# zdebruine/MMVAE

Hardware: AMD Instinct MI355X
Metric: cells/sec per MMVAE train step (higher is better)
Workload: dtype f32; 1 GPU; c2: 2-modality MMVAE train step, 20000 genes each, latent 128, K=1, batch 512/GPU, adversarial=False; global_batch=512, parallelism=dp1, exchange=none

## Files before the change

__graft_entry__.py:

```python
import os
import subprocess
import sys

ROOT = os.path.dirname(os.path.abspath(__file__))
if ROOT not in sys.path:
    sys.path.insert(0, ROOT)


def build() -> None:
    csrc = os.path.join(ROOT, "mmvae_amd", "csrc")
    subprocess.run(["make", "-C", csrc, "-j4"], check=True)
    from mmvae_amd import _lib

    lib = _lib.load()
    assert lib.mmvae_abi_version() >= 1 and lib.mmvae_build_arch() == b"gfx950"
    from mmvae_amd import _stats_lib

    stats = _stats_lib.load_stats()
    assert stats.mmvae_stats_abi_version() == _stats_lib.STATS_ABI_VERSION and stats.mmvae_stats_build_arch() == b"gfx950"
    from mmvae_amd import _disc_lib

    disc = _disc_lib.load_disc()
    assert disc.mmvae_disc_abi_version() == _disc_lib.DISC_ABI_VERSION and disc.mmvae_disc_build_arch() == b"gfx950"
    from mmvae_amd import _umap_lib

    um = _umap_lib.load_umap()
    assert um.mmvae_umap_abi_version() == _umap_lib.UMAP_ABI_VERSION and um.mmvae_umap_build_arch() == b"gfx950"
    from mmvae_amd import _hist_lib

    hist = _hist_lib.load_hist()
    assert hist.mmvae_hist_abi_version() == _hist_lib.HIST_ABI_VERSION and hist.mmvae_hist_build_arch() == b"gfx950"
    from mmvae_amd import _prep_lib

    prep = _prep_lib.load_prep()
    assert prep.mmvae_prep_abi_version() == _prep_lib.PREP_ABI_VERSION and prep.mmvae_prep_build_arch() == b"gfx950"
    from mmvae_amd import data

    assert data.feed_lib().mmvae_feed_abi_version() == 3
    import mmvae_amd.models
    import mmvae_amd.modules
    import mmvae_amd.engine


def smoke() -> None:
    import torch

    assert torch.cuda.is_available(), "smoke() needs a GPU"
    from mmvae_amd import _lib

    _lib.load()
# ... 12 lines not shown
```

mmvae_amd/csrc/elbo_optim.hip:

```cpp
#include "common.h"

namespace {

__global__ __launch_bounds__(256) void reparam_kl_fwd_kernel(int B, int Z, int K, const float* __restrict__ mu,
                                                             const float* __restrict__ a_raw,
                                                             const float* __restrict__ eps, float var_eps,
                                                             float* __restrict__ std_out, float* __restrict__ z_out,
                                                             float* __restrict__ kl_row, float* __restrict__ stat_row) {
    const int lane = threadIdx.x & 63;
    const int b = blockIdx.x * 4 + (threadIdx.x >> 6);
    if (b >= B) return;
    float kl = 0.f, smu = 0.f, svar = 0.f;
    for (int j = lane; j < Z; j += 64) {
        const int64_t o = (int64_t)b * Z + j;
        const float m = mu[o];
        const float v = expf(a_raw[o]) + var_eps;
        const float s = sqrtf(v);
        if (std_out) std_out[o] = s;
        const float vr = s * s;
        kl += 0.5f * (vr + m * m - 1.f - logf(vr));
        smu += m;
        svar += vr;
        if (z_out)
            for (int k = 0; k < K; ++k) {
// ... 366 lines not shown
        for (int64_t i = threadIdx.x; i < n; i += 1024) s += (double)row[i];
        __syncthreads();
        red[threadIdx.x] = s;
        __syncthreads();
        for (int st = 512; st >= 1; st >>= 1) {
            if ((int)threadIdx.x < st) red[threadIdx.x] += red[threadIdx.x + st];
            __syncthreads();
        }
        const float r = (float)red[0];
        if (threadIdx.x == 0 && out_each) out_each[h] = r;
        total = h == 0 ? r : total + r;
    }
    if (threadIdx.x == 0 && out_total) out_total[0] = total;
}

constexpr int64_t SQN_CHUNK = 1 << 16;

__device__ __forceinline__ float sqnorm_chunk(int64_t n, const float* __restrict__ g, int64_t chunk, float* red) {
    const int64_t beg = chunk * SQN_CHUNK;
    int64_t end = beg + SQN_CHUNK;
    if (end > n) end = n;
    float s = 0.f;
    const bool vec = ((reinterpret_cast<uintptr_t>(g) & 15u) == 0);
    if (vec) {
        const int64_t nv = (end - beg) / 4;
        const f32x4* gv = reinterpret_cast<const f32x4*>(g + beg);
        float s0 = 0.f, s1 = 0.f, s2 = 0.f, s3 = 0.f;
        int64_t i = threadIdx.x;
        for (; i + 7 * 256 < nv; i += 8 * 256) {
            f32x4 v[8];
#pragma unroll
            for (int u = 0; u < 8; ++u) v[u] = gv[i + u * 256];
#pragma unroll
            for (int u = 0; u < 8; ++u) {
                s0 += v[u].x * v[u].x;
                s1 += v[u].y * v[u].y;
                s2 += v[u].z * v[u].z;
                s3 += v[u].w * v[u].w;
            }
        }
        for (; i < nv; i += 256) {
            const f32x4 v = gv[i];
            s0 += v.x * v.x;
            s1 += v.y * v.y;
            s2 += v.z * v.z;
            s3 += v.w * v.w;
        }
        s = (s0 + s1) + (s2 + s3);
        for (int64_t i = beg + nv * 4 + threadIdx.x; i < end; i += 256) s += g[i] * g[i];
    } else {
        for (int64_t i = beg + threadIdx.x; i < end; i += 256) s += g[i] * g[i];
    }
    s = wave_sum(s);
    __syncthreads();
    if ((threadIdx.x & 63) == 0) red[threadIdx.x >> 6] = s;
    __syncthreads();
    return (red[0] + red[1]) + (red[2] + red[3]);
}

__global__ __launch_bounds__(256) void sqnorm_kernel(int64_t n, const float* __restrict__ g,
                                                     float* __restrict__ partials) {
    __shared__ float red[4];
    const float s = sqnorm_chunk(n, g, blockIdx.x, red);
    if (threadIdx.x == 0) partials[blockIdx.x] = s;
}

__device__ __forceinline__ void adam_prepare_body(int64_t np, const float* partials, float max_norm, float grad_scale,
                                                  float beta1, float beta2, float* __restrict__ state, unsigned flags,
                                                  double* red) {
    double s = 0.0;
    if (flags & MMVAE_PREPARE_NORM)
        for (int64_t i = threadIdx.x; i < np; i += 256) s += (double)partials[i];
    red[threadIdx.x] = s;
    __syncthreads();
    if (threadIdx.x == 0) {
        double t = 0.0;
        if (flags & MMVAE_PREPARE_NORM)
            for (int i = 0; i < 256; ++i) t += red[i];
        adam_state_finish(state, t, flags, max_norm, grad_scale, beta1, beta2);
    }
}

__global__ __launch_bounds__(256) void adam_prepare_kernel(int64_t np, const float* __restrict__ partials,
                                                           float max_norm, float grad_scale, float beta1, float beta2,
                                                           float* __restrict__ state, unsigned flags) {
    __shared__ double red[256];
    adam_prepare_body(np, partials, max_norm, grad_scale, beta1, beta2, state, flags, red);
}

struct SqRanges {
    const float* g[4];
    int64_t n[4];
    int nb[4];
    int nr;
};
// ... 12 lines not shown
    }
    const float s = sqnorm_chunk(r.n[k], r.g[k], b, red);
    if (threadIdx.x == 0) {
        partials[blockIdx.x] = s;
        __threadfence();
        last = atomicAdd(ticket, 1u) == gridDim.x - 1;
    }
    __syncthreads();
    if (!last) return;
    if (threadIdx.x == 0) *ticket = 0u;
    __threadfence();
    adam_prepare_body(np_all, const_cast<const float*>(reinterpret_cast<const volatile float*>(partials_all)), max_norm,
                      grad_scale, beta1, beta2, state, flags, dred);
}

#ifndef MMVAE_ADAM_NT
#define MMVAE_ADAM_NT 1
#endif
__device__ __forceinline__ void adam_one(float& p, float g, float& m, float& v, float gmul, float wd, float b1, float b2,
                                         float step_size, float inv_bc2_sqrt, float eps, float cv = 0.f) {
    const float gs = g * gmul;
    const float gc = (gs != gs ? gs : fminf(fmaxf(gs, -cv), cv)) + wd * p;
    g = g * gmul + wd * p;
    if (cv > 0.f) g = gc;
    m = m + (1.f - b1) * (g - m);
    v = b2 * v + (1.f - b2) * g * g;
    const float denom = sqrtf(v) * inv_bc2_sqrt + eps;
    p = p - step_size * (m / denom);
}

__device__ __forceinline__ float mul_uncontracted(float a, float b) {
#pragma clang fp contract(off)
    return a * b;
}
__device__ __forceinline__ void adam_hyper(const float* __restrict__ hyper, float& lr, float& wd, float& decay) {
    decay = 1.f;
    lr = hyper[0];
    wd = hyper[1];
    if (hyper[2] != 0.f) {
        decay = 1.f - mul_uncontracted(lr, wd);
        wd = 0.f;
    }
}
__device__ __forceinline__ void adam_elem(float& p, float g, float& m, float& v, float gmul, float wd, float decay,
                                          float b1, float b2, float step_size, float inv_bc2_sqrt, float eps, float cv) {
    p = mul_uncontracted(p, decay);
    adam_one(p, g, m, v, gmul, wd, b1, b2, step_size, inv_bc2_sqrt, eps, cv);
}

__device__ __forceinline__ void adam_step_body(int64_t n, float* __restrict__ p, const float* __restrict__ g,
                                               float* __restrict__ m, float* __restrict__ v,
                                               const float* __restrict__ state, const float* __restrict__ hyper,
                                               float b1, float b2, float eps, float grad_scale, int vec, int copy_n,
                                               const float* copy_src, float* copy_dst) {
    if (copy_n > 0 && blockIdx.x == 0)
        for (int i = threadIdx.x; i < copy_n; i += blockDim.x) copy_dst[i] = copy_src[i];
    float lr, wd, decay;
    adam_hyper(hyper, lr, wd, decay);
    const float gmul = state[2] * grad_scale;
    const float step_size = lr / state[3];
    const float inv_bc2_sqrt = 1.f / sqrtf(state[4]);
    const float cv = state[5];
    const int64_t stride = (int64_t)gridDim.x * blockDim.x;
    const int64_t tid0 = (int64_t)blockIdx.x * blockDim.x + threadIdx.x;
    if (vec) {
        const int64_t nv = n / 4;
        f32x4* pv = reinterpret_cast<f32x4*>(p);
        const f32x4* gv = reinterpret_cast<const f32x4*>(g);
        f32x4* mv = reinterpret_cast<f32x4*>(m);
        f32x4* vv = reinterpret_cast<f32x4*>(v);
        for (int64_t i = tid0; i < nv; i += stride) {
#if MMVAE_ADAM_NT
            f32x4 pp = MMVAE_ADAM_NT == 2 ? __builtin_nontemporal_load(pv + i) : pv[i];
            f32x4 gg = __builtin_nontemporal_load(gv + i), mm = __builtin_nontemporal_load(mv + i),
                  vw = __builtin_nontemporal_load(vv + i);
#else
            f32x4 pp = pv[i], gg = gv[i], mm = mv[i], vw = vv[i];
#endif
#pragma unroll
            for (int e = 0; e < 4; ++e) {
                float pe = pp[e], me = mm[e], ve = vw[e];
                adam_elem(pe, gg[e], me, ve, gmul, wd, decay, b1, b2, step_size, inv_bc2_sqrt, eps, cv);
                pp[e] = pe;
                mm[e] = me;
                vw[e] = ve;
            }
#if MMVAE_ADAM_NT == 2
            __builtin_nontemporal_store(pp, pv + i);
#else
            pv[i] = pp;
#endif
#if MMVAE_ADAM_NT
            __builtin_nontemporal_store(mm, mv + i);
            __builtin_nontemporal_store(vw, vv + i);
#else
            mv[i] = mm;
            vv[i] = vw;
#endif
        }
        for (int64_t i = nv * 4 + tid0; i < n; i += stride)
            adam_elem(p[i], g[i], m[i], v[i], gmul, wd, decay, b1, b2, step_size, inv_bc2_sqrt, eps, cv);
    } else {
        for (int64_t i = tid0; i < n; i += stride)
            adam_elem(p[i], g[i], m[i], v[i], gmul, wd, decay, b1, b2, step_size, inv_bc2_sqrt, eps, cv);
    }
}

__global__ __launch_bounds__(256) void adam_step_hp_kernel(int64_t n, float* __restrict__ p, const float* __restrict__ g,
                                                           float* __restrict__ m, float* __restrict__ v,
                                                           const float* __restrict__ state,
                                                           const float* __restrict__ hyper, float b1, float b2, float eps,
                                                           float grad_scale, int vec, int copy_n, const float* copy_src,
                                                           float* copy_dst) {
    adam_step_body(n, p, g, m, v, state, hyper, b1, b2, eps, grad_scale, vec, copy_n, copy_src, copy_dst);
}

constexpr int ADAM_WIDE_LDS = 84 * 1024;
__global__ __launch_bounds__(1024) void adam_step_wide_hp_kernel(int64_t n, float* __restrict__ p,
                                                                 const float* __restrict__ g, float* __restrict__ m,
                                                                 float* __restrict__ v, const float* __restrict__ state,
// ... 1003 lines not shown
```

mmvae_amd/engine.py:

```python
from __future__ import annotations

import os
from dataclasses import dataclass
from typing import Dict, List, Optional

import torch

from . import _lib, dist as mdist, rng
from .constants import REGISTRY_KEYS as RK
from .engine_adv import PlanAdversaries
from .engine_common import ACC, NN, NT, RELU, SQ_FUSED_SLOTS, TN, _LayerRef, _PlaneBuf, _block_decline, _p
from .engine_cond import CondProgram
from .engine_emit import PlanEmit
from .engine_run import PlanRun
from .modules.base.components import Adversarial, FCBlock, _identity
from .optim import HipAdam

MAX_POINTER_PLANS = 8
SIDE_MAX_ROWS = 640
ADV_DW_CAP = 170


@dataclass(frozen=True)
class EngineSettings:
# ... 2 lines not shown
    planes: bool = True
    side_dw: int = 125
    side_dw2: int = 185
    side_dw_dp: int = 125
    side_dw_any: bool = False
    prefetch_adv: int = 86
    cond_batched: bool = True
    prefetch: int = 128
    adv_fused: bool = True
    adv_aside: int = 2
    dp_overlap: Optional[bool] = None
    dp_shard: bool = True
    dp_kernels: str = "auto"
    dp_sim_world: int = 0
    dp_autotune_force: bool = False
    stamps: bool = False

    @staticmethod
    def from_env() -> "EngineSettings":
        e = os.environ.get
        ov = e("MMVAE_DP_OVERLAP", "")
        kernels = e("MMVAE_DP_KERNELS", "auto")
        if kernels not in ("auto", "dynamic", "persistent"):
            raise _lib.HipLibraryError(f"MMVAE_DP_KERNELS={kernels!r}: dynamic | persistent | auto")
        return EngineSettings(
            conditionals=e("MMVAE_ENGINE_CONDITIONALS", "1") != "0", graphs=e("MMVAE_NO_GRAPH", "0") == "0",
            planes=e("MMVAE_PLANES", "1") != "0", side_dw=int(e("MMVAE_SIDE_DW", "125")),
            side_dw2=int(e("MMVAE_SIDE_DW2", "185")), side_dw_dp=int(e("MMVAE_SIDE_DW_DP", "125")),
            side_dw_any=e("MMVAE_SIDE_DW_ANY", "0") != "0", prefetch=int(e("MMVAE_PREFETCH", "128")),
            cond_batched=e("MMVAE_COND_BATCHED", "1") != "0", prefetch_adv=int(e("MMVAE_PREFETCH_ADV", "86")),
            adv_fused=e("MMVAE_ADV_FUSED", "1") != "0",
            adv_aside=int(e("MMVAE_ADV_ASIDE", "2")),
            dp_overlap=None if ov == "" else ov != "0", dp_shard=e("MMVAE_DP_SHARD", "1") != "0", dp_kernels=kernels,
            dp_sim_world=int(e("MMVAE_DP_SIM_WORLD", "0")), dp_autotune_force=e("MMVAE_DP_AUTOTUNE_FORCE", "0") != "0",
            stamps=e("MMVAE_STAMPS", "0") == "1")


FORK_VALIDATED_RUNTIMES = ("7.0.",)


def concurrent_streams(device, n: int, pool: int = 12) -> list:
    main = torch.cuda.current_stream(device)
    spin = 400_000
    out = []
    for _ in range(pool):
        c = torch.cuda.Stream(device=device)
        torch.cuda.synchronize(device)
        t0, t1, m0, m1 = (torch.cuda.Event(enable_timing=True) for _ in range(4))
        ev = torch.cuda.Event()
# ... 665 lines not shown
        self._dirty: List = []
        self._sq_used: Dict[int, int] = {}
        self._sq_cover: Dict[int, list] = {}
        self._mask_layers: List = []
        self._gemm_jobs: List = []
        self._sum_jobs: List = []
        self._sum_keep: List = []
        self._job_tables: List = []
        self._ws_bytes = 0
        self._slab_floats = 0
        self._graphs: Optional[list] = None
        self._probe_next = None
        self.probe = None
        self.probe_meta: Dict[str, dict] = {}
        self._forked = False
        self._events: List = []
        self._runs = 0
        self.exp_norm_log = None
        self._x_split_jobs: List = []
        self._defer_next_dw = False
        self._deferred_dw = None
        self._fcws_bytes = 0
        self._defer_id = 0
        self.x_fp32_dw1 = False
        self.adv_grad_into: Dict[int, torch.Tensor] = {}
        self.n_adv = 0
        self._label_ring = None
        self._log_cache: Dict[tuple, list] = {}
        self.metrics = eng.buf("metrics", (256,))
        self.rng_state = rng.state(eng.device)
# ... 401 lines not shown
            if early and j == self.n_expert_enc:
                self._begin_exchange(self.opt_vae)
        self._mark("backward chain done")

    def _emit_optimisers(self):
        eng, lib, L = self.eng, self.lib, self.layout
        self.log_buf = torch.zeros(256, dtype=torch.float32, device=eng.device)

        def emit_log_copy():
            self._emit(lib.mmvae_axpby, 256, 1.0, _p(self.metrics), 0.0, _p(self.log_buf))

        early = eng.overlap
        deferred, self._deferred_dw = self._deferred_dw, None
        late_branch = bool(L.late and deferred is not None and self.cond is None)
        start = len(self._cur)
        self.optimizer(self.opt_vae, self.clip_vae, exchange="wait" if early else "inline", join=not late_branch)
        self.log_norm(self.opt_vae, "grad_norms/vae")
        if late_branch:
            calls = self._take(start)
            self._fork()
            (layout, M, N, Kk, A, lda, Bm, ldb, Cm, ldc), dwp = deferred
            self._probe_next = "enc_l1_dw"
            if not self._fuse_sqnorm(layout, M, N, Kk, 1.0, A, lda, Bm, ldb, Cm, ldc, None, 0, side_cap=L.late_cap,
                                     on_side=False, planes=dwp):
                self.gemm(*deferred[0], side=True, planes=dwp)
            self._probe_next = None
            self._branch(eng.side_stream, calls + [c for c in [self._mark_call("VAE optimiser done (branch)")] if c])
        elif deferred is not None:
            self._probe_next = "enc_l1_dw" if L.big else None
            self.gemm(*deferred[0], side=True, planes=deferred[1])
            self._probe_next = None
# ... 54 lines not shown
```

mmvae_amd/engine_emit.py:

```python
from __future__ import annotations

import ctypes as C
from typing import Optional

import torch

from . import _lib, dist as mdist
from .engine_common import ACC, NN, NT, RAW, RELU, SLACK, SQ_FUSED_SLOTS, TN, _LayerRef, _NOPL, _PlaneBuf, _p, _planes_desc, _s
from .optim import HipAdam


class PlanEmit:
    def _emit(self, fn, *args, probe=None):
        lib_fn = fn

        def call():
            rc = lib_fn(*args, _s())
            if rc != 0:
                raise _lib.HipLibraryError(f"{lib_fn.__name__} failed with code {rc}")

        self._cur.append(self._probed(probe[0], probe[1], call) if probe else call)

    def _mark_call(self, name: str):
        if not self.eng.stamps:
            return None
        slot = len(self.stamp_names)
        self.stamp_names.append(name)
        buf = self.eng.buf("debug.stamps", (256,), torch.int64)
        lib = self.lib

        def call():
            lib.mmvae_debug_stamp(buf.data_ptr(), slot, _s())

        return call

    def _mark(self, name: str):
        c = self._mark_call(name)
        if c is not None:
            self._cur.append(c)

    def _probed(self, tag, work, call, **meta):
        if tag is None:
            return call
        plan = self
        self.probe_meta[tag] = dict(meta, work=work)

        def wrapped():
            pr = plan.probe
# ... 76 lines not shown
        plan, lib = self, self.lib
        ap, bp = (planes[0].args() if planes and planes[0] else _NOPL), (planes[1].args() if planes and planes[1] else _NOPL)
        tag, self._probe_next = self._probe_next, None
        sq_args = sq if sq else (None, 0)

        def launch_gemm():
            ws = (plan.ws.data_ptr(), plan.ws.numel() * 4) if use_ws else (None, 0)
            c_ptr = _p(Cm) if Cm is not None else plan.slab.data_ptr()
            rc = lib.mmvae_gemm_planes_f32(layout, M, N, K, alpha, _p(A), lda, *ap, _p(Bm), ldb, *bp, c_ptr, ldc,
                                           _p(bias), flags | SLACK, sk, *ws, *sq_args, _s())
            if rc != 0:
                raise _lib.HipLibraryError(f"GEMM launch failed with code {rc} (layout {layout}, {M}x{N}x{K})")

        launch = self._probed(tag, 2.0 * M * N * K, launch_gemm, bound="mfma", cus=cap, planes=_planes_desc(planes),
                              shape=f"{('NT', 'NN', 'TN')[layout]} {M}x{N}x{K}" + (f" split-K {sk}" if sk > 1 else ""))
        if not cap:
            self._cur.append(launch)
            return
        if stream is not None:
            self._fork(stream)

        def call():
            lib.mmvae_gemm_set_workgroup_cap(cap)
            try:
                if stream is not None:
                    with torch.cuda.stream(stream):
                        launch()
                else:
                    launch()
            finally:
                lib.mmvae_gemm_set_workgroup_cap(0)

        self._cur.append(call)

    def _queue_gemm(self, layout, M, N, K, alpha, A, lda, Bm, ldb, Cm, ldc, bias, flags) -> bool:
# ... 29 lines not shown
            tile = self._plan_tile(layout, M, N, K)[0]
            job = _lib.GemmJob(_p(A), _p(Bm), _p(Cm), _p(bias), lda, ldb, ldc, layout, M, N, K, float(alpha), int(flags), 0, 0)
            if tile != 2 or not self.lib.mmvae_gemm_batch_job_ok(C.addressof(job)):
                return False
            arr.append(job)
            self._sum_keep.append((A, Bm, Cm, bias))
        self._emit_gemm_batch(arr)
        return True

    def _flush_gemms(self):
        if self._gemm_jobs:
            self._emit_gemm_batch(self._gemm_jobs)
            self._gemm_jobs = []

    def _emit_gemm_batch(self, jobs):
        table = (_lib.GemmJob * len(jobs))(*jobs)
        total = C.c_int(0)
        _lib.check(self.lib.mmvae_gemm_batch_prepare(len(jobs), C.addressof(table), C.byref(total)), "mmvae_gemm_batch_prepare")
        self._emit(self.lib.mmvae_gemm_batch_f32, len(jobs), self._upload_table(table), total.value)

    def _upload_table(self, table) -> int:
        t = torch.frombuffer(bytearray(bytes(table)), dtype=torch.uint8).to(self.eng.device)
        self._job_tables.append(t)
        return t.data_ptr()

    def gemm(self, layout, M, N, K, A, lda, Bm, ldb, Cm, ldc, bias=None, flags=0, alpha=1.0, side=False, planes=None):
        if side and self._queue_gemm(layout, M, N, K, alpha, A, lda, Bm, ldb, Cm, ldc, bias, flags):
            return
        sk = self._plan_gemm(layout, M, N, K)
        if side and sk > 1 and not (flags & ~ACC) and bias is None:
# ... 30 lines not shown
        job = self._x_split_jobs.pop(0)
        return _lib.SplitJob(*job[:4], _lib.Planes(*job[4:]))

    def _fork(self, stream=None):
        side = stream if stream is not None else self.eng.side_stream
        self._edge(None, side)
        self._forked = True
        if side not in self._dirty:
            self._dirty.append(side)

    def _join(self, only=None):
        for side in self._dirty:
            if only is None or side is only:
                self._edge(side, None)
        self._dirty = [] if only is None else [s for s in self._dirty if s is not only]

    def _take(self, start: int) -> list:
        calls = self._cur[start:]
        del self._cur[start:]
        return calls

    def _branch(self, stream, calls):
        if not calls:
            return

        def call():
            with torch.cuda.stream(stream):
                for c in calls:
                    c()

        self._cur.append(call)
        if stream not in self._dirty:
            self._dirty.append(stream)

    def _next_defer_id(self) -> int:
        self._defer_id += 1
        return self._defer_id

    def _defer_sum(self, src, n_parts, part_stride, rows, cols, ld_src, dst, ld_dst, alpha=1.0, flags=0):
        self._sum_jobs.append(_lib.SumJob(_p(src), _p(dst), part_stride, ld_src, ld_dst, n_parts, rows, cols, float(alpha),
                                          int(flags), 0))
        self._sum_keep.append((src, dst))

    def _flush_sums(self):
        self._flush_gemms()
        if not self._sum_jobs:
            return
        arr = (_lib.SumJob * len(self._sum_jobs))(*self._sum_jobs)
        self._emit(self.lib.mmvae_sum_parts_batch, len(self._sum_jobs), self._upload_table(arr),
                   max(int(j.rows) * int(j.cols) for j in self._sum_jobs))
        self._sum_jobs = []

    def gemm_raw(self, layout, M, N, K, A, lda, Bm, ldb, planes=None) -> int:
        sk = self._plan_gemm(layout, M, N, K)
        self._slab_floats = max(self._slab_floats, sk * M * N)
        self._gemm_launch(layout, M, N, K, 1.0, A, lda, Bm, ldb, None, N, None, RAW, sk=sk, planes=planes)
        return sk

    def fwd_layer(self, tag: str, l: _LayerRef, cur: torch.Tensor, ld_cur: int, rows: int, training: bool = True,
                  mask_tag: Optional[str] = None, mask_stream: Optional[int] = None, planes_out: Optional[_PlaneBuf] = None,
                  split_job=None, slabs_from: Optional[torch.Tensor] = None):
        eng = self.eng
# ... 174 lines not shown
        plan = self
        self._fcws_bytes = max(self._fcws_bytes, self.lib.mmvae_fc_workspace_bytes(rows, N))
        own_ws = self._bias_partials(rows, N, dbias) if dbias is not None else None

        def call():
            ws = own_ws if own_ws is not None else plan.fcws
            rc = plan.lib.mmvae_fc_epilogue_bwd(rows, N, _p(din), N, 1, _p(addend), None, _p(row_scale), None, 0.0, 0, None, None,
                                                None, None, None, 0, _p(dz_out), N, _p(dbias) if own_ws is None else None,
                                                None, None, ws.data_ptr(), ws.numel() * 4, None, _s())
            if rc != 0:
                raise _lib.HipLibraryError(f"mmvae_fc_epilogue_bwd (column sum) failed with code {rc}")

        self._cur.append(call)

    def optimizer(self, opt: HipAdam, max_norm: float, advance: bool = True, step: bool = True, exchange: str = "inline",
                  join: bool = True, tail_copy=None):
        if join:
            self._join()
        self._flush_sums()
        a = opt.arena
        g = opt.param_groups[0]
        b1, b2 = g["betas"]
        gs = 1.0 / self.eng.world
        npart = self.lib.mmvae_sqnorm_partials(a.numel)
        sh = a.shard(self.eng.shard_sim_world or self.eng.world, mdist.rank()) if (
            self.eng.shard and opt is self.opt_exp and self.cond is None
                                                       and exchange in ("inline", "deferred")
                                                       and opt.reducer is not None) else None
        if sh is not None:
            return self._optimizer_sharded(opt, sh, max_norm, advance, step, exchange)
        if (opt.reducer is not None or self.eng.overlap) and exchange != "done":
# ... 12 lines not shown
        ranges, pos = [], 0
        for off, n in cover + [(a.numel, 0)]:
            if off > pos:
                ranges.append((pos, off - pos))
            pos = max(pos, off + n)
        buf = self.eng.sq_buffer(opt) if cover else opt.partials
        slot = self._sq_used.pop(id(opt)) if cover else 0
        nparts = [self.lib.mmvae_sqnorm_partials(n) for _, n in ranges]
        npart = slot + sum(nparts)
        assert npart <= buf.numel()
        if 1 <= len(ranges) <= 4 and opt.reducer is None and not self.eng.overlap:
            gp = (C.c_void_p * len(ranges))(*[a.grad.data_ptr() + 4 * o for o, _ in ranges])
            ln = (C.c_int64 * len(ranges))(*[n for _, n in ranges])
            ticket = self.eng.buf(f"sqticket.{id(opt)}", (1,), torch.int32)
            self._sum_keep.append((gp, ln, ticket))
            self._emit(self.lib.mmvae_grad_sqnorm_ranges_prepare, len(ranges), C.addressof(gp), C.addressof(ln),
                       buf.data_ptr() + 4 * slot, _p(ticket), npart, _p(buf), max_norm, gs, b1, b2, _p(opt.state_dev), flags)
        else:
            for (o, n), k in zip(ranges, nparts):
                self._emit(self.lib.mmvae_grad_sqnorm, n, a.grad.data_ptr() + 4 * o, buf.data_ptr() + 4 * slot)
                slot += k
            self._emit(self.lib.mmvae_adam_prepare, npart, _p(buf), max_norm, gs, b1, b2, _p(opt.state_dev), flags)
        pr = ("adam_expert", 28.0 * a.numel) if opt is self.opt_exp else None
        if step and tail_copy is not None:
            self._emit(self.lib.mmvae_adam_step_copy_hp, a.numel, _p(a.data), _p(a.grad), _p(a.exp_avg), _p(a.exp_avg_sq),
                       _p(opt.state_dev), _p(opt.hyper_dev), b1, b2, g["eps"], gs, tail_copy[0], _p(tail_copy[1]),
                       _p(tail_copy[2]), probe=pr)
        elif step:
            self._emit(self.lib.mmvae_adam_step_hp, a.numel, _p(a.data), _p(a.grad), _p(a.exp_avg), _p(a.exp_avg_sq),
                       _p(opt.state_dev), _p(opt.hyper_dev), b1, b2, g["eps"], gs, probe=pr)
        if step and pr:
            self.probe_meta["adam_expert"].update(bound="hbm", cus=0, shape=f"{a.numel} parameters, 28 B each")

    def _optimizer_sharded(self, opt: HipAdam, sh, max_norm, advance, step, exchange):
        a, g, lib = opt.arena, opt.param_groups[0], self.lib
        b1, b2 = g["betas"]
        gs = 1.0 / self.eng.world
        per, lo, n_loc = sh
        W = self.eng.world
        sim = bool(self.eng.shard_sim_world)
        mine = self.eng.buf(f"shard.sq.{id(opt)}", (1,))
        allsq = self.eng.buf(f"shard.allsq.{id(opt)}", (W,))
        self.shard_info = dict(per=per, lo=lo, n_loc=n_loc, mine=mine, allsq=allsq, sim=sim)
        opt.sharded = not sim
        self._cut(("rs_" + exchange, opt))
        if n_loc > 0:
            np_loc = int(lib.mmvae_sqnorm_partials(n_loc))
# ... 31 lines not shown
```

Before: 584,400 cells/s.

## Fuse expert grad-norm into VAE norm launch and fuse Adam prepare with step

Adds a tail library with two kernels. One computes squared-norm partials for the VAE and expert optimizers in a single launch. The other runs the norm reduction, clip preparation and the Adam update (plus an optional tail copy) in one persistent-grid kernel that uses a ticket to synchronise. The engine retroactively upgrades the earlier VAE norm launch when ordering conditions allow, and falls back when late gradient writes or open branches are detected. This removes several small launches and serialisation points at the end of the step. In exchange it adds bookkeeping that is fragile with respect to stream ordering.

```diff
diff --git a/__graft_entry__.py b/__graft_entry__.py
--- a/__graft_entry__.py
+++ b/__graft_entry__.py
@@ -34,6 +34,10 @@
 
     prep = _prep_lib.load_prep()
     assert prep.mmvae_prep_abi_version() == _prep_lib.PREP_ABI_VERSION and prep.mmvae_prep_build_arch() == b"gfx950"
+    from mmvae_amd import _tail_lib
+
+    tail = _tail_lib.load_tail()
+    assert tail.mmvae_tail_abi_version() == _tail_lib.TAIL_ABI_VERSION and tail.mmvae_tail_build_arch() == b"gfx950"
     from mmvae_amd import data
 
     assert data.feed_lib().mmvae_feed_abi_version() == 3
diff --git a/include/mmvae_tail.h b/include/mmvae_tail.h
--- /dev/null
+++ b/include/mmvae_tail.h
@@ -0,0 +1,42 @@
+#ifndef MMVAE_TAIL_H
+#define MMVAE_TAIL_H
+
+#include <stddef.h>
+#include <stdint.h>
+
+#ifdef __cplusplus
+extern "C" {
+#endif
+
+#ifndef MMVAE_OK
+typedef void* mmvae_stream_t;
+#define MMVAE_OK 0
+#define MMVAE_ERR_ARG 1
+#define MMVAE_ERR_LAUNCH 2
+#endif
+#ifndef MMVAE_PREPARE_NORM
+#define MMVAE_PREPARE_NORM 1u
+#define MMVAE_PREPARE_ADVANCE 2u
+#endif
+
+#define MMVAE_TAIL_ABI_VERSION 1
+int mmvae_tail_abi_version(void);
+const char* mmvae_tail_build_arch(void);
+
+#define MMVAE_TAIL_MAX_RANGES 4
+#define MMVAE_TAIL_MAX_WORKGROUPS 65536
+
+int mmvae_tail_sqnorm_two(int n_ranges_a, const float* const* grads_a, const int64_t* lens_a, float* partials_a,
+                          unsigned* ticket, int64_t n_partials_all, const float* partials_all, float max_norm,
+                          float grad_scale, float beta1, float beta2, float* state, unsigned flags, int n_ranges_b,
+                          const float* const* grads_b, const int64_t* lens_b, float* partials_b, mmvae_stream_t stream);
+
+int mmvae_tail_adam_fused(int64_t n, float* param, const float* grad, float* exp_avg, float* exp_avg_sq, float* state,
+                          const float* hyper, float beta1, float beta2, float eps, float grad_scale, int copy_n,
+                          const float* copy_src, float* copy_dst, int64_t np, const float* partials, float max_norm,
+                          unsigned flags, unsigned* ticket, int workgroups, mmvae_stream_t stream);
+
+#ifdef __cplusplus
+}
+#endif
+#endif
diff --git a/mmvae_amd/_tail_lib.py b/mmvae_amd/_tail_lib.py
--- /dev/null
+++ b/mmvae_amd/_tail_lib.py
@@ -0,0 +1,58 @@
+from __future__ import annotations
+
+import ctypes as C
+import os
+from typing import Optional
+
+from ._lib import ERR_ARG, ERR_LAUNCH, OK, HipLibraryError, check
+
+_HERE = os.path.dirname(os.path.abspath(__file__))
+TAIL_LIB_PATH = os.path.join(_HERE, "csrc", "libmmvae_tail.so")
+
+TAIL_ABI_VERSION = 1
+TAIL_MAX_RANGES = 4
+TAIL_MAX_WORKGROUPS = 65536
+
+_p = C.c_void_p
+_i = C.c_int
+_l = C.c_int64
+_f = C.c_float
+_u = C.c_uint
+
+TAIL_PROTOTYPES = {
+    "mmvae_tail_abi_version": (_i, []),
+    "mmvae_tail_build_arch": (C.c_char_p, []),
+    "mmvae_tail_sqnorm_two": (_i, [_i, _p, _p, _p, _p, _l, _p, _f, _f, _f, _f, _p, _u, _i, _p, _p, _p, _p]),
+    "mmvae_tail_adam_fused": (_i, [_l, _p, _p, _p, _p, _p, _p, _f, _f, _f, _f, _i, _p, _p, _l, _p, _f, _u, _p, _i, _p]),
+}
+
+_tail: Optional[C.CDLL] = None
+
+
+def load_tail() -> C.CDLL:
+    global _tail
+    if _tail is not None:
+        return _tail
+    import torch
+
+    if not os.path.exists(TAIL_LIB_PATH):
+        raise HipLibraryError(
+            f"{TAIL_LIB_PATH} not found: build it with `make -C mmvae_amd/csrc` (or __graft_entry__.build()). "
+            "mmvae_amd has no non-HIP execution path for device tensors."
+        )
+    try:
+        lib = C.CDLL(TAIL_LIB_PATH)
+    except OSError as e:
+        raise HipLibraryError(f"could not load {TAIL_LIB_PATH}: {e}") from e
+    for name, (res, args) in TAIL_PROTOTYPES.items():
+        try:
+            fn = getattr(lib, name)
+        except AttributeError as e:
+            raise HipLibraryError(f"{TAIL_LIB_PATH} does not export {name}") from e
+        fn.restype = res
+        fn.argtypes = args
+    if lib.mmvae_tail_abi_version() != TAIL_ABI_VERSION:
+        raise HipLibraryError(f"{TAIL_LIB_PATH} has ABI {lib.mmvae_tail_abi_version()}, this binding was written "
+                              f"against {TAIL_ABI_VERSION}: rebuild it")
+    _tail = lib
+    return lib
diff --git a/mmvae_amd/csrc/adam_dev.h b/mmvae_amd/csrc/adam_dev.h
--- /dev/null
+++ b/mmvae_amd/csrc/adam_dev.h
@@ -0,0 +1,145 @@
+#pragma once
+#include "common.h"
+
+constexpr int64_t SQN_CHUNK = 1 << 16;
+
+__device__ __forceinline__ float sqnorm_chunk(int64_t n, const float* __restrict__ g, int64_t chunk, float* red) {
+    const int64_t beg = chunk * SQN_CHUNK;
+    int64_t end = beg + SQN_CHUNK;
+    if (end > n) end = n;
+    float s = 0.f;
+    const bool vec = ((reinterpret_cast<uintptr_t>(g) & 15u) == 0);
+    if (vec) {
+        const int64_t nv = (end - beg) / 4;
+        const f32x4* gv = reinterpret_cast<const f32x4*>(g + beg);
+        float s0 = 0.f, s1 = 0.f, s2 = 0.f, s3 = 0.f;
+        int64_t i = threadIdx.x;
+        for (; i + 7 * 256 < nv; i += 8 * 256) {
+            f32x4 v[8];
+#pragma unroll
+            for (int u = 0; u < 8; ++u) v[u] = gv[i + u * 256];
+#pragma unroll
+            for (int u = 0; u < 8; ++u) {
+                s0 += v[u].x * v[u].x;
+                s1 += v[u].y * v[u].y;
+                s2 += v[u].z * v[u].z;
+                s3 += v[u].w * v[u].w;
+            }
+        }
+        for (; i < nv; i += 256) {
+            const f32x4 v = gv[i];
+            s0 += v.x * v.x;
+            s1 += v.y * v.y;
+            s2 += v.z * v.z;
+            s3 += v.w * v.w;
+        }
+        s = (s0 + s1) + (s2 + s3);
+        for (int64_t i = beg + nv * 4 + threadIdx.x; i < end; i += 256) s += g[i] * g[i];
+    } else {
+        for (int64_t i = beg + threadIdx.x; i < end; i += 256) s += g[i] * g[i];
+    }
+    s = wave_sum(s);
+    __syncthreads();
+    if ((threadIdx.x & 63) == 0) red[threadIdx.x >> 6] = s;
+    __syncthreads();
+    return (red[0] + red[1]) + (red[2] + red[3]);
+}
+
+__device__ __forceinline__ void adam_prepare_body(int64_t np, const float* partials, float max_norm, float grad_scale,
+                                                  float beta1, float beta2, float* __restrict__ state, unsigned flags,
+                                                  double* red) {
+    double s = 0.0;
+    if (flags & MMVAE_PREPARE_NORM)
+        for (int64_t i = threadIdx.x; i < np; i += 256) s += (double)partials[i];
+    red[threadIdx.x] = s;
+    __syncthreads();
+    if (threadIdx.x == 0) {
+        double t = 0.0;
+        if (flags & MMVAE_PREPARE_NORM)
+            for (int i = 0; i < 256; ++i) t += red[i];
+        adam_state_finish(state, t, flags, max_norm, grad_scale, beta1, beta2);
+    }
+}
+
+#ifndef MMVAE_ADAM_NT
+#define MMVAE_ADAM_NT 1
+#endif
+__device__ __forceinline__ void adam_one(float& p, float g, float& m, float& v, float gmul, float wd, float b1, float b2,
+                                         float step_size, float inv_bc2_sqrt, float eps, float cv = 0.f) {
+    const float gs = g * gmul;
+    const float gc = (gs != gs ? gs : fminf(fmaxf(gs, -cv), cv)) + wd * p;
+    g = g * gmul + wd * p;
+    if (cv > 0.f) g = gc;
+    m = m + (1.f - b1) * (g - m);
+    v = b2 * v + (1.f - b2) * g * g;
+    const float denom = sqrtf(v) * inv_bc2_sqrt + eps;
+    p = p - step_size * (m / denom);
+}
+
+__device__ __forceinline__ float mul_uncontracted(float a, float b) {
+#pragma clang fp contract(off)
+    return a * b;
+}
+__device__ __forceinline__ void adam_hyper(const float* __restrict__ hyper, float& lr, float& wd, float& decay) {
+    decay = 1.f;
+    lr = hyper[0];
+    wd = hyper[1];
+    if (hyper[2] != 0.f) {
+        decay = 1.f - mul_uncontracted(lr, wd);
+        wd = 0.f;
+    }
+}
+__device__ __forceinline__ void adam_elem(float& p, float g, float& m, float& v, float gmul, float wd, float decay,
+                                          float b1, float b2, float step_size, float inv_bc2_sqrt, float eps, float cv) {
+    p = mul_uncontracted(p, decay);
+    adam_one(p, g, m, v, gmul, wd, b1, b2, step_size, inv_bc2_sqrt, eps, cv);
+}
+
+__device__ __forceinline__ void adam_elem_loop(int64_t n, float* __restrict__ p, const float* __restrict__ g,
+                                               float* __restrict__ m, float* __restrict__ v, float gmul, float wd,
+                                               float decay, float b1, float b2, float step_size, float inv_bc2_sqrt,
+                                               float eps, float cv, int vec) {
+    const int64_t stride = (int64_t)gridDim.x * blockDim.x;
+    const int64_t tid0 = (int64_t)blockIdx.x * blockDim.x + threadIdx.x;
+    if (vec) {
+        const int64_t nv = n / 4;
+        f32x4* pv = reinterpret_cast<f32x4*>(p);
+        const f32x4* gv = reinterpret_cast<const f32x4*>(g);
+        f32x4* mv = reinterpret_cast<f32x4*>(m);
+        f32x4* vv = reinterpret_cast<f32x4*>(v);
+        for (int64_t i = tid0; i < nv; i += stride) {
+#if MMVAE_ADAM_NT
+            f32x4 pp = MMVAE_ADAM_NT == 2 ? __builtin_nontemporal_load(pv + i) : pv[i];
+            f32x4 gg = __builtin_nontemporal_load(gv + i), mm = __builtin_nontemporal_load(mv + i),
+                  vw = __builtin_nontemporal_load(vv + i);
+#else
+            f32x4 pp = pv[i], gg = gv[i], mm = mv[i], vw = vv[i];
+#endif
+#pragma unroll
+            for (int e = 0; e < 4; ++e) {
+                float pe = pp[e], me = mm[e], ve = vw[e];
+                adam_elem(pe, gg[e], me, ve, gmul, wd, decay, b1, b2, step_size, inv_bc2_sqrt, eps, cv);
+                pp[e] = pe;
+                mm[e] = me;
+                vw[e] = ve;
+            }
+#if MMVAE_ADAM_NT == 2
+            __builtin_nontemporal_store(pp, pv + i);
+#else
+            pv[i] = pp;
+#endif
+#if MMVAE_ADAM_NT
+            __builtin_nontemporal_store(mm, mv + i);
+            __builtin_nontemporal_store(vw, vv + i);
+#else
+            mv[i] = mm;
+            vv[i] = vw;
+#endif
+        }
+        for (int64_t i = nv * 4 + tid0; i < n; i += stride)
+            adam_elem(p[i], g[i], m[i], v[i], gmul, wd, decay, b1, b2, step_size, inv_bc2_sqrt, eps, cv);
+    } else {
+        for (int64_t i = tid0; i < n; i += stride)
+            adam_elem(p[i], g[i], m[i], v[i], gmul, wd, decay, b1, b2, step_size, inv_bc2_sqrt, eps, cv);
+    }
+}
diff --git a/mmvae_amd/csrc/elbo_optim.hip b/mmvae_amd/csrc/elbo_optim.hip
--- a/mmvae_amd/csrc/elbo_optim.hip
+++ b/mmvae_amd/csrc/elbo_optim.hip
@@ -1,4 +1,5 @@
 #include "common.h"
+#include "adam_dev.h"
 
 namespace {
 
@@ -404,71 +405,11 @@
     if (threadIdx.x == 0 && out_total) out_total[0] = total;
 }
 
-constexpr int64_t SQN_CHUNK = 1 << 16;
-
-__device__ __forceinline__ float sqnorm_chunk(int64_t n, const float* __restrict__ g, int64_t chunk, float* red) {
-    const int64_t beg = chunk * SQN_CHUNK;
-    int64_t end = beg + SQN_CHUNK;
-    if (end > n) end = n;
-    float s = 0.f;
-    const bool vec = ((reinterpret_cast<uintptr_t>(g) & 15u) == 0);
-    if (vec) {
-        const int64_t nv = (end - beg) / 4;
-        const f32x4* gv = reinterpret_cast<const f32x4*>(g + beg);
-        float s0 = 0.f, s1 = 0.f, s2 = 0.f, s3 = 0.f;
-        int64_t i = threadIdx.x;
-        for (; i + 7 * 256 < nv; i += 8 * 256) {
-            f32x4 v[8];
-#pragma unroll
-            for (int u = 0; u < 8; ++u) v[u] = gv[i + u * 256];
-#pragma unroll
-            for (int u = 0; u < 8; ++u) {
-                s0 += v[u].x * v[u].x;
-                s1 += v[u].y * v[u].y;
-                s2 += v[u].z * v[u].z;
-                s3 += v[u].w * v[u].w;
-            }
-        }
-        for (; i < nv; i += 256) {
-            const f32x4 v = gv[i];
-            s0 += v.x * v.x;
-            s1 += v.y * v.y;
-            s2 += v.z * v.z;
-            s3 += v.w * v.w;
-        }
-        s = (s0 + s1) + (s2 + s3);
-        for (int64_t i = beg + nv * 4 + threadIdx.x; i < end; i += 256) s += g[i] * g[i];
-    } else {
-        for (int64_t i = beg + threadIdx.x; i < end; i += 256) s += g[i] * g[i];
-    }
-    s = wave_sum(s);
-    __syncthreads();
-    if ((threadIdx.x & 63) == 0) red[threadIdx.x >> 6] = s;
-    __syncthreads();
-    return (red[0] + red[1]) + (red[2] + red[3]);
-}
-
 __global__ __launch_bounds__(256) void sqnorm_kernel(int64_t n, const float* __restrict__ g,
                                                      float* __restrict__ partials) {
     __shared__ float red[4];
     const float s = sqnorm_chunk(n, g, blockIdx.x, red);
     if (threadIdx.x == 0) partials[blockIdx.x] = s;
-}
-
-__device__ __forceinline__ void adam_prepare_body(int64_t np, const float* partials, float max_norm, float grad_scale,
-                                                  float beta1, float beta2, float* __restrict__ state, unsigned flags,
-                                                  double* red) {
-    double s = 0.0;
-    if (flags & MMVAE_PREPARE_NORM)
-        for (int64_t i = threadIdx.x; i < np; i += 256) s += (double)partials[i];
-    red[threadIdx.x] = s;
-    __syncthreads();
-    if (threadIdx.x == 0) {
-        double t = 0.0;
-        if (flags & MMVAE_PREPARE_NORM)
-            for (int i = 0; i < 256; ++i) t += red[i];
-        adam_state_finish(state, t, flags, max_norm, grad_scale, beta1, beta2);
-    }
 }
 
 __global__ __launch_bounds__(256) void adam_prepare_kernel(int64_t np, const float* __restrict__ partials,
@@ -511,40 +452,6 @@
                       grad_scale, beta1, beta2, state, flags, dred);
 }
 
-#ifndef MMVAE_ADAM_NT
-#define MMVAE_ADAM_NT 1
-#endif
-__device__ __forceinline__ void adam_one(float& p, float g, float& m, float& v, float gmul, float wd, float b1, float b2,
-                                         float step_size, float inv_bc2_sqrt, float eps, float cv = 0.f) {
-    const float gs = g * gmul;
-    const float gc = (gs != gs ? gs : fminf(fmaxf(gs, -cv), cv)) + wd * p;
-    g = g * gmul + wd * p;
-    if (cv > 0.f) g = gc;
-    m = m + (1.f - b1) * (g - m);
-    v = b2 * v + (1.f - b2) * g * g;
-    const float denom = sqrtf(v) * inv_bc2_sqrt + eps;
-    p = p - step_size * (m / denom);
-}
-
-__device__ __forceinline__ float mul_uncontracted(float a, float b) {
-#pragma clang fp contract(off)
-    return a * b;
-}
-__device__ __forceinline__ void adam_hyper(const float* __restrict__ hyper, float& lr, float& wd, float& decay) {
-    decay = 1.f;
-    lr = hyper[0];
-    wd = hyper[1];
-    if (hyper[2] != 0.f) {
-        decay = 1.f - mul_uncontracted(lr, wd);
-        wd = 0.f;
-    }
-}
-__device__ __forceinline__ void adam_elem(float& p, float g, float& m, float& v, float gmul, float wd, float decay,
-                                          float b1, float b2, float step_size, float inv_bc2_sqrt, float eps, float cv) {
-    p = mul_uncontracted(p, decay);
-    adam_one(p, g, m, v, gmul, wd, b1, b2, step_size, inv_bc2_sqrt, eps, cv);
-}
-
 __device__ __forceinline__ void adam_step_body(int64_t n, float* __restrict__ p, const float* __restrict__ g,
                                                float* __restrict__ m, float* __restrict__ v,
                                                const float* __restrict__ state, const float* __restrict__ hyper,
@@ -558,49 +465,7 @@
     const float step_size = lr / state[3];
     const float inv_bc2_sqrt = 1.f / sqrtf(state[4]);
     const float cv = state[5];
-    const int64_t stride = (int64_t)gridDim.x * blockDim.x;
-    const int64_t tid0 = (int64_t)blockIdx.x * blockDim.x + threadIdx.x;
-    if (vec) {
-        const int64_t nv = n / 4;
-        f32x4* pv = reinterpret_cast<f32x4*>(p);
-        const f32x4* gv = reinterpret_cast<const f32x4*>(g);
-        f32x4* mv = reinterpret_cast<f32x4*>(m);
-        f32x4* vv = reinterpret_cast<f32x4*>(v);
-        for (int64_t i = tid0; i < nv; i += stride) {
-#if MMVAE_ADAM_NT
-            f32x4 pp = MMVAE_ADAM_NT == 2 ? __builtin_nontemporal_load(pv + i) : pv[i];
-            f32x4 gg = __builtin_nontemporal_load(gv + i), mm = __builtin_nontemporal_load(mv + i),
-                  vw = __builtin_nontemporal_load(vv + i);
-#else
-            f32x4 pp = pv[i], gg = gv[i], mm = mv[i], vw = vv[i];
-#endif
-#pragma unroll
-            for (int e = 0; e < 4; ++e) {
-                float pe = pp[e], me = mm[e], ve = vw[e];
-                adam_elem(pe, gg[e], me, ve, gmul, wd, decay, b1, b2, step_size, inv_bc2_sqrt, eps, cv);
-                pp[e] = pe;
-                mm[e] = me;
-                vw[e] = ve;
-            }
-#if MMVAE_ADAM_NT == 2
-            __builtin_nontemporal_store(pp, pv + i);
-#else
-            pv[i] = pp;
-#endif
-#if MMVAE_ADAM_NT
-            __builtin_nontemporal_store(mm, mv + i);
-            __builtin_nontemporal_store(vw, vv + i);
-#else
-            mv[i] = mm;
-            vv[i] = vw;
-#endif
-        }
-        for (int64_t i = nv * 4 + tid0; i < n; i += stride)
-            adam_elem(p[i], g[i], m[i], v[i], gmul, wd, decay, b1, b2, step_size, inv_bc2_sqrt, eps, cv);
-    } else {
-        for (int64_t i = tid0; i < n; i += stride)
-            adam_elem(p[i], g[i], m[i], v[i], gmul, wd, decay, b1, b2, step_size, inv_bc2_sqrt, eps, cv);
-    }
+    adam_elem_loop(n, p, g, m, v, gmul, wd, decay, b1, b2, step_size, inv_bc2_sqrt, eps, cv, vec);
 }
 
 __global__ __launch_bounds__(256) void adam_step_hp_kernel(int64_t n, float* __restrict__ p, const float* __restrict__ g,
diff --git a/mmvae_amd/csrc/optim_tail.hip b/mmvae_amd/csrc/optim_tail.hip
--- /dev/null
+++ b/mmvae_amd/csrc/optim_tail.hip
@@ -0,0 +1,142 @@
+#include "adam_dev.h"
+#include "../../include/mmvae_tail.h"
+
+namespace {
+
+struct SqRanges {
+    const float* g[MMVAE_TAIL_MAX_RANGES];
+    int64_t n[MMVAE_TAIL_MAX_RANGES];
+    int nb[MMVAE_TAIL_MAX_RANGES];
+    int nr;
+};
+
+__global__ __launch_bounds__(256) void sqnorm_two_kernel(SqRanges ra, SqRanges rb, int nblk_a, float* __restrict__ partials_a,
+                                                         float* __restrict__ partials_b, unsigned* __restrict__ ticket,
+                                                         int64_t np_all, const float* partials_all, float max_norm,
+                                                         float grad_scale, float beta1, float beta2,
+                                                         float* __restrict__ state, unsigned flags) {
+    __shared__ float red[4];
+    __shared__ double dred[256];
+    __shared__ int last;
+    const bool is_b = (int)blockIdx.x >= nblk_a;
+    const SqRanges& r = is_b ? rb : ra;
+    const int slot = is_b ? (int)blockIdx.x - nblk_a : (int)blockIdx.x;
+    int b = slot, k = 0;
+    while (k + 1 < r.nr && b >= r.nb[k]) {
+        b -= r.nb[k];
+        ++k;
+    }
+    const float s = sqnorm_chunk(r.n[k], r.g[k], b, red);
+    if (is_b) {
+        if (threadIdx.x == 0) partials_b[slot] = s;
+        return;
+    }
+    if (threadIdx.x == 0) {
+        partials_a[slot] = s;
+        __threadfence();
+        last = atomicAdd(ticket, 1u) == (unsigned)nblk_a - 1u;
+    }
+    __syncthreads();
+    if (!last) return;
+    if (threadIdx.x == 0) *ticket = 0u;
+    __threadfence();
+    adam_prepare_body(np_all, const_cast<const float*>(reinterpret_cast<const volatile float*>(partials_all)), max_norm,
+                      grad_scale, beta1, beta2, state, flags, dred);
+}
+
+constexpr int STATE_WRITTEN = 5;
+
+__global__ __launch_bounds__(256) void adam_fused_kernel(int64_t n, float* __restrict__ p, const float* __restrict__ g,
+                                                         float* __restrict__ m, float* __restrict__ v, float* state,
+                                                         const float* __restrict__ hyper, float b1, float b2, float eps,
+                                                         float grad_scale, int vec, int copy_n, const unsigned* copy_src,
+                                                         unsigned* copy_dst, int64_t np, const float* __restrict__ partials,
+                                                         float max_norm, unsigned flags, unsigned* __restrict__ ticket) {
+    __shared__ double dred[256];
+    __shared__ float st[MMVAE_ADAM_STATE_FLOATS];
+    __shared__ int last;
+    if (threadIdx.x < MMVAE_ADAM_STATE_FLOATS) st[threadIdx.x] = state[threadIdx.x];
+    __syncthreads();
+    adam_prepare_body(np, partials, max_norm, grad_scale, b1, b2, st, flags, dred);
+    __syncthreads();
+    float lr, wd, decay;
+    adam_hyper(hyper, lr, wd, decay);
+    const float gmul = st[2] * grad_scale;
+    const float step_size = lr / st[3];
+    const float inv_bc2_sqrt = 1.f / sqrtf(st[4]);
+    const float cv = st[5];
+    adam_elem_loop(n, p, g, m, v, gmul, wd, decay, b1, b2, step_size, inv_bc2_sqrt, eps, cv, vec);
+
+    __syncthreads();
+    if (threadIdx.x == 0) last = atomicAdd(ticket, 1u) == gridDim.x - 1;
+    __syncthreads();
+    if (!last) return;
+    if (threadIdx.x == 0) {
+        *ticket = 0u;
+        for (int i = 0; i < STATE_WRITTEN; ++i) state[i] = st[i];
+    }
+    const unsigned* sw = reinterpret_cast<const unsigned*>(state);
+    for (int i = threadIdx.x; i < copy_n; i += 256) {
+        const ptrdiff_t d = (copy_src + i) - sw;
+        copy_dst[i] = (d >= 0 && d < STATE_WRITTEN) ? __float_as_uint(st[d]) : copy_src[i];
+    }
+}
+
+bool fill_ranges(SqRanges& r, int n_ranges, const float* const* grads, const int64_t* lens, int& total) {
+    r.nr = n_ranges;
+    total = 0;
+    for (int i = 0; i < n_ranges; ++i) {
+        if (!grads[i] || lens[i] <= 0) return false;
+        const int64_t nb = ceil_div_l(lens[i], SQN_CHUNK);
+        if (nb > (1 << 24)) return false;
+        r.g[i] = grads[i];
+        r.n[i] = lens[i];
+        r.nb[i] = (int)nb;
+        total += (int)nb;
+    }
+    return true;
+}
+
+}
+
+extern "C" int mmvae_tail_abi_version(void) { return MMVAE_TAIL_ABI_VERSION; }
+extern "C" const char* mmvae_tail_build_arch(void) { return "gfx950"; }
+
+extern "C" int mmvae_tail_sqnorm_two(int n_ranges_a, const float* const* grads_a, const int64_t* lens_a, float* partials_a,
+                                     unsigned* ticket, int64_t n_partials_all, const float* partials_all, float max_norm,
+                                     float grad_scale, float beta1, float beta2, float* state, unsigned flags,
+                                     int n_ranges_b, const float* const* grads_b, const int64_t* lens_b, float* partials_b,
+                                     mmvae_stream_t stream) {
+    if (n_ranges_a < 1 || n_ranges_a > MMVAE_TAIL_MAX_RANGES || !grads_a || !lens_a || !partials_a || !ticket ||
+        !partials_all || !state || n_partials_all <= 0)
+        return MMVAE_ERR_ARG;
+    if (n_ranges_b < 0 || n_ranges_b > MMVAE_TAIL_MAX_RANGES) return MMVAE_ERR_ARG;
+    if (n_ranges_b > 0 && (!grads_b || !lens_b || !partials_b)) return MMVAE_ERR_ARG;
+    SqRanges ra = {}, rb = {};
+    int total_a = 0, total_b = 0;
+    if (!fill_ranges(ra, n_ranges_a, grads_a, lens_a, total_a)) return MMVAE_ERR_ARG;
+    if (!fill_ranges(rb, n_ranges_b, grads_b, lens_b, total_b)) return MMVAE_ERR_ARG;
+    MMVAE_LAUNCH(sqnorm_two_kernel, dim3((unsigned)(total_a + total_b)), dim3(256), 0, (hipStream_t)stream, ra, rb, total_a,
+                 partials_a, partials_b, ticket, n_partials_all, partials_all, max_norm, grad_scale, beta1, beta2, state,
+                 flags | MMVAE_PREPARE_NORM);
+    MMVAE_LAUNCH_CHECK();
+    return MMVAE_OK;
+}
+
+extern "C" int mmvae_tail_adam_fused(int64_t n, float* param, const float* grad, float* exp_avg, float* exp_avg_sq,
+                                     float* state, const float* hyper, float beta1, float beta2, float eps,
+                                     float grad_scale, int copy_n, const float* copy_src, float* copy_dst, int64_t np,
+                                     const float* partials, float max_norm, unsigned flags, unsigned* ticket,
+                                     int workgroups, mmvae_stream_t stream) {
+    if (n <= 0 || !param || !grad || !exp_avg || !exp_avg_sq || !state || !hyper || !ticket) return MMVAE_ERR_ARG;
+    if (copy_n < 0 || copy_n > 65536 || (copy_n > 0 && (!copy_src || !copy_dst))) return MMVAE_ERR_ARG;
+    if (np < 0 || ((flags & MMVAE_PREPARE_NORM) && np > 0 && !partials)) return MMVAE_ERR_ARG;
+    if (workgroups <= 0 || workgroups > MMVAE_TAIL_MAX_WORKGROUPS) return MMVAE_ERR_ARG;
+    const int vec = aligned16(param) && aligned16(grad) && aligned16(exp_avg) && aligned16(exp_avg_sq);
+    MMVAE_LAUNCH(adam_fused_kernel, dim3((unsigned)workgroups), dim3(256), 0, (hipStream_t)stream, n, param, grad, exp_avg,
+                 exp_avg_sq, state, hyper, beta1, beta2, eps, grad_scale, vec, copy_n,
+                 reinterpret_cast<const unsigned*>(copy_src), reinterpret_cast<unsigned*>(copy_dst), np, partials, max_norm,
+                 flags, ticket);
+    MMVAE_LAUNCH_CHECK();
+    return MMVAE_OK;
+}
diff --git a/mmvae_amd/engine.py b/mmvae_amd/engine.py
--- a/mmvae_amd/engine.py
+++ b/mmvae_amd/engine.py
@@ -40,6 +40,8 @@
     dp_kernels: str = "auto"
     dp_sim_world: int = 0
     dp_autotune_force: bool = False
+    tail_fused: bool = True
+    tail_wg_per_cu: int = 2
     stamps: bool = False
 
     @staticmethod
@@ -59,6 +61,7 @@
             adv_aside=int(e("MMVAE_ADV_ASIDE", "2")),
             dp_overlap=None if ov == "" else ov != "0", dp_shard=e("MMVAE_DP_SHARD", "1") != "0", dp_kernels=kernels,
             dp_sim_world=int(e("MMVAE_DP_SIM_WORLD", "0")), dp_autotune_force=e("MMVAE_DP_AUTOTUNE_FORCE", "0") != "0",
+            tail_fused=e("MMVAE_TAIL_FUSED", "1") != "0", tail_wg_per_cu=int(e("MMVAE_TAIL_WG_PER_CU", "2")),
             stamps=e("MMVAE_STAMPS", "0") == "1")
 
 
@@ -754,6 +757,9 @@
         self.probe = None
         self.probe_meta: Dict[str, dict] = {}
         self._forked = False
+        self._branch_open: set = set()
+        self._tail_host = None
+        self.emitted: List[str] = []
         self._events: List = []
         self._runs = 0
         self.exp_norm_log = None
@@ -1185,7 +1191,8 @@
         deferred, self._deferred_dw = self._deferred_dw, None
         late_branch = bool(L.late and deferred is not None and self.cond is None)
         start = len(self._cur)
-        self.optimizer(self.opt_vae, self.clip_vae, exchange="wait" if early else "inline", join=not late_branch)
+        self.optimizer(self.opt_vae, self.clip_vae, exchange="wait" if early else "inline", join=not late_branch,
+                       norm_stream=eng.side_stream if late_branch else None)
         self.log_norm(self.opt_vae, "grad_norms/vae")
         if late_branch:
             calls = self._take(start)
diff --git a/mmvae_amd/engine_emit.py b/mmvae_amd/engine_emit.py
--- a/mmvae_amd/engine_emit.py
+++ b/mmvae_amd/engine_emit.py
@@ -5,7 +5,7 @@
 
 import torch
 
-from . import _lib, dist as mdist
+from . import _lib, _tail_lib, dist as mdist
 from .engine_common import ACC, NN, NT, RAW, RELU, SLACK, SQ_FUSED_SLOTS, TN, _LayerRef, _NOPL, _PlaneBuf, _p, _planes_desc, _s
 from .optim import HipAdam
 
@@ -19,6 +19,7 @@
             if rc != 0:
                 raise _lib.HipLibraryError(f"{lib_fn.__name__} failed with code {rc}")
 
+        self.emitted.append(fn.__name__)
         self._cur.append(self._probed(probe[0], probe[1], call) if probe else call)
 
     def _mark_call(self, name: str):
@@ -32,6 +33,7 @@
         def call():
             lib.mmvae_debug_stamp(buf.data_ptr(), slot, _s())
 
+        call.is_mark = True
         return call
 
     def _mark(self, name: str):
@@ -138,11 +140,15 @@
 
         launch = self._probed(tag, 2.0 * M * N * K, launch_gemm, bound="mfma", cus=cap, planes=_planes_desc(planes),
                               shape=f"{('NT', 'NN', 'TN')[layout]} {M}x{N}x{K}" + (f" split-K {sk}" if sk > 1 else ""))
+        if not sq and self._tail_host is not None and Cm is not None and self.eng.locate_grad(Cm) is not None:
+            self._tail_host["late_writes"] = True
         if not cap:
             self._cur.append(launch)
             return
         if stream is not None:
             self._fork(stream)
+            if not sq:
+                self._branch_open.add(id(stream))
 
         def call():
             lib.mmvae_gemm_set_workgroup_cap(cap)
@@ -202,6 +208,8 @@
             self._gemm_jobs = []
 
     def _emit_gemm_batch(self, jobs):
+        if self._tail_host is not None:
+            self._tail_host["late_writes"] = True
         table = (_lib.GemmJob * len(jobs))(*jobs)
         total = C.c_int(0)
         _lib.check(self.lib.mmvae_gemm_batch_prepare(len(jobs), C.addressof(table), C.byref(total)), "mmvae_gemm_batch_prepare")
@@ -262,6 +270,7 @@
             if only is None or side is only:
                 self._edge(side, None)
         self._dirty = [] if only is None else [s for s in self._dirty if s is not only]
+        self._branch_open = {id(s) for s in self._dirty if id(s) in self._branch_open}
 
     def _take(self, start: int) -> list:
         calls = self._cur[start:]
@@ -278,6 +287,8 @@
                     c()
 
         self._cur.append(call)
+        if not all(getattr(c, "is_mark", False) for c in calls):
+            self._branch_open.add(id(stream))
         if stream not in self._dirty:
             self._dirty.append(stream)
 
@@ -294,6 +305,8 @@
         self._flush_gemms()
         if not self._sum_jobs:
             return
+        if self._tail_host is not None:
+            self._tail_host["late_writes"] = True
         arr = (_lib.SumJob * len(self._sum_jobs))(*self._sum_jobs)
         self._emit(self.lib.mmvae_sum_parts_batch, len(self._sum_jobs), self._upload_table(arr),
                    max(int(j.rows) * int(j.cols) for j in self._sum_jobs))
@@ -498,7 +511,7 @@
         self._cur.append(call)
 
     def optimizer(self, opt: HipAdam, max_norm: float, advance: bool = True, step: bool = True, exchange: str = "inline",
-                  join: bool = True, tail_copy=None):
+                  join: bool = True, tail_copy=None, norm_stream=None):
         if join:
             self._join()
         self._flush_sums()
@@ -541,8 +554,17 @@
             ln = (C.c_int64 * len(ranges))(*[n for _, n in ranges])
             ticket = self.eng.buf(f"sqticket.{id(opt)}", (1,), torch.int32)
             self._sum_keep.append((gp, ln, ticket))
-            self._emit(self.lib.mmvae_grad_sqnorm_ranges_prepare, len(ranges), C.addressof(gp), C.addressof(ln),
-                       buf.data_ptr() + 4 * slot, _p(ticket), npart, _p(buf), max_norm, gs, b1, b2, _p(opt.state_dev), flags)
+            host, self._tail_host = (self._tail_host, None) if opt is self.opt_exp else (None, self._tail_host)
+            if host is not None and step and host["ordered"] and not host["late_writes"]:
+                self._emit_tail_fused(opt, host, (len(ranges), C.addressof(gp), C.addressof(ln), buf.data_ptr() + 4 * slot),
+                                      npart, buf, max_norm, flags, tail_copy)
+                return
+            norm_args = (len(ranges), C.addressof(gp), C.addressof(ln), buf.data_ptr() + 4 * slot, _p(ticket), npart, _p(buf),
+                         max_norm, gs, b1, b2, _p(opt.state_dev), flags)
+            if opt is self.opt_vae and self.eng.settings.tail_fused and not self.has_adv:
+                self._emit_norm_host(norm_args, norm_stream)
+            else:
+                self._emit(self.lib.mmvae_grad_sqnorm_ranges_prepare, *norm_args)
         else:
             for (o, n), k in zip(ranges, nparts):
                 self._emit(self.lib.mmvae_grad_sqnorm, n, a.grad.data_ptr() + 4 * o, buf.data_ptr() + 4 * slot)
@@ -558,6 +580,41 @@
                        _p(opt.state_dev), _p(opt.hyper_dev), b1, b2, g["eps"], gs, probe=pr)
         if step and pr:
             self.probe_meta["adam_expert"].update(bound="hbm", cus=0, shape=f"{a.numel} parameters, 28 B each")
+
+    def _emit_norm_host(self, norm_args, norm_stream):
+        ordered = all(s is norm_stream or id(s) not in self._branch_open for s in self._dirty)
+        host = dict(b=None, ordered=ordered, late_writes=False, index=len(self.emitted))
+        self._tail_host = host
+        self.emitted.append("mmvae_grad_sqnorm_ranges_prepare")
+        lib = self.lib
+
+        def call():
+            if host["b"] is None:
+                rc, name = lib.mmvae_grad_sqnorm_ranges_prepare(*norm_args, _s()), "mmvae_grad_sqnorm_ranges_prepare"
+            else:
+                rc, name = _tail_lib.load_tail().mmvae_tail_sqnorm_two(*norm_args, *host["b"], _s()), "mmvae_tail_sqnorm_two"
+            if rc != 0:
+                raise _lib.HipLibraryError(f"{name} failed with code {rc}")
+
+        self._cur.append(call)
+
+    def _emit_tail_fused(self, opt: HipAdam, host, b_ranges, npart, buf, max_norm, flags, tail_copy):
+        a, g = opt.arena, opt.param_groups[0]
+        b1, b2 = g["betas"]
+        gs = 1.0 / self.eng.world
+        tail = _tail_lib.load_tail()
+        host["b"] = b_ranges
+        self.emitted[host["index"]] = "mmvae_tail_sqnorm_two"
+        ticket = self.eng.buf(f"tailticket.{id(opt)}", (1,), torch.int32)
+        self._sum_keep.append(ticket)
+        cus = torch.cuda.get_device_properties(self.eng.device).multi_processor_count
+        workgroups = max(1, min(self.eng.settings.tail_wg_per_cu * cus, (a.numel + 1023) // 1024))
+        n_copy, src, dst = tail_copy if tail_copy is not None else (0, None, None)
+        self._emit(tail.mmvae_tail_adam_fused, a.numel, _p(a.data), _p(a.grad), _p(a.exp_avg), _p(a.exp_avg_sq),
+                   _p(opt.state_dev), _p(opt.hyper_dev), b1, b2, g["eps"], gs, n_copy, _p(src), _p(dst), npart, _p(buf),
+                   max_norm, flags, _p(ticket), workgroups,
+                   probe=("adam_expert", 28.0 * a.numel))
+        self.probe_meta["adam_expert"].update(bound="hbm", cus=0, shape=f"{a.numel} parameters, 28 B each")
 
     def _optimizer_sharded(self, opt: HipAdam, sh, max_norm, advance, step, exchange):
         a, g, lib = opt.arena, opt.param_groups[0], self.lib
```

After: 588,000 cells/s, median of 5. About the same (+0.6%).
